# tszalay/poreseq

Measured on AMD Instinct MI355X. Metric: kb consensus refined/sec at 10x coverage, higher is better.
Workload: dtype f64; 1 GPU; poreseq consensus, 10 kb region, 10x synthetic coverage (BASELINE configs[1]), full Mutate.py schedule per region; a step is 280 independent regions per GPU = 14 lock-step batches; the batches of the timed steps run step by step (a step's batches all finish before the next step's start) through 14 batch slots (host threads) per GPU; marshalling + H2D of the events, host greedy steps and D2H inside; region_bases=10000, events=10, regions_per_gpu=280, batches_in_flight=14, step_barrier=True, parallelism=280 regions x 1 GPU(s), 14 host thread(s) per GPU, no data-path collective

## Files before the change

### poreseq_amd/csrc/ps_api.cpp

```cpp
#include <algorithm>
#include <cmath>
#include <cstring>
#include <memory>

#include "ps_host.h"
#include "ps_sw.h"

using namespace ps;

struct ps_align { Align a; };
struct ps_muts { std::vector<Mut> v; };
struct ps_seqs { std::vector<std::string> v; };
struct ps_rng { RandState* s = nullptr; ~ps_rng() { if (s) rand_state_free(s); } };

#define NEED_RT()            \
    Runtime* rt = nullptr;   \
    PS_TRY(runtime(&rt))

extern "C" {

const char* ps_last_error(void) { return last_error(); }
const char* ps_backend_name(void) { return "hip-gfx950"; }
int ps_info(char* out, int64_t cap) {
    if (!out || cap <= 0) return fail(PS_ERR_BAD_ARG, "ps_info");
// ... 458 lines not shown
    std::vector<std::unique_ptr<ps_seqs>> s(n);
    std::vector<VitReq> rq(n);
    for (int i = 0; i < n; i++) { s[i].reset(new ps_seqs()); rq[i].a = as[i]; rq[i].rng = (rng && rng[i]) ? rng[i]->s : nullptr; rq[i].out = &s[i]->v; }
    VitCall call;
    call.nkeep = nkeep; call.skip = skip; call.stay = stay; call.mmin = mmin; call.mmax = mmax;
    PS_TRY(viterbi_mutate(nullptr, call, rq.data(), rq.size()));
    for (int i = 0; i < n; i++) out[i] = s[i].release();
    return PS_OK;
}

int ps_swfull(const char* s1, int64_t n1, const char* s2, int64_t n2, int32_t* score, double* acc,
              int32_t* i1, int32_t* i2, int64_t cap, int64_t* np) {
    if (!s1 || !s2 || n1 < 0 || n2 < 0 || !np) return fail(PS_ERR_BAD_ARG, "ps_swfull");
    NEED_RT();
    int sc = 0; double ac = 0;
    std::vector<int> a, b;
    PS_TRY(sw_device(rt, std::string(s1, n1), std::string(s2, n2), &sc, &ac, &a, &b));
    if ((int64_t)a.size() > cap) return fail(PS_ERR_BAD_ARG, "ps_swfull: index capacity too small");
    if (score) *score = sc;
    if (acc) *acc = ac;
    for (size_t k = 0; k < a.size(); k++) { if (i1) i1[k] = a[k]; if (i2) i2[k] = b[k]; }
    *np = (int64_t)a.size();
    return PS_OK;
}
int ps_batch_sw_summary(int64_t n, const char* const* seq1, const int64_t* n1, const char* const* seq2, const int64_t* n2,
                        ps_sw_summary* out) {
    if (n < 0 || (n && (!seq1 || !n1 || !seq2 || !n2 || !out))) return fail(PS_ERR_BAD_ARG, "ps_batch_sw_summary");
    for (int64_t k = 0; k < n; k++)
        if (n1[k] < 0 || n2[k] < 0 || (n1[k] && !seq1[k]) || (n2[k] && !seq2[k])) return fail(PS_ERR_BAD_ARG, "ps_batch_sw_summary: bad pair");
    if (!n) return PS_OK;
    NEED_RT();
    std::vector<std::string> s(2 * (size_t)n);
    SwInput in;
    for (int64_t k = 0; k < n; k++) {
        if (n1[k]) s[2 * k].assign(seq1[k], (size_t)n1[k]);
        if (n2[k]) s[2 * k + 1].assign(seq2[k], (size_t)n2[k]);
    }
    for (int64_t k = 0; k < n; k++) in.push_back({&s[2 * k], &s[2 * k + 1]});
    std::vector<SwResult> res;
    PS_TRY(sw_summaries(rt, in, &res));
    for (int64_t k = 0; k < n; k++) {
        const SwResult& r = res[k];
        ps_sw_summary& o = out[k];
        o.score = r.score; o.n_pairs = r.n_pairs; o.n_match = r.n_match;
        o.first1 = r.first1; o.first2 = r.first2; o.last1 = r.last1; o.last2 = r.last2;
        o.gap1 = r.gap1; o.gap2 = r.gap2;
        o.accuracy = r.accuracy;
    }
    return PS_OK;
}
int ps_seq_to_states(const char* seq, int64_t n, int32_t* st, int64_t* ns) {
    if (!seq || n < 0 || !ns) return fail(PS_ERR_BAD_ARG, "ps_seq_to_states");
    std::vector<int> v = states_of(std::string(seq, n));
    if (st) std::copy(v.begin(), v.end(), st);
    *ns = (int64_t)v.size();
    return PS_OK;
}

int ps_debug_sw_band(int64_t* out) {
    if (!out) return fail(PS_ERR_BAD_ARG, "ps_debug_sw_band");
    sw_band_counters(out);
    return PS_OK;
}
int ps_debug_posterior(ps_align* a, int32_t e, double* main, double* stay) {
    if (!a || e < 0 || e >= a->a.E || !main) return fail(PS_ERR_BAD_ARG, "ps_debug_posterior");
    if (!a->a.nonfinite.empty()) return fail(PS_ERR_BAD_ARG, "ps_debug_posterior: " + a->a.nonfinite);
    NEED_RT();
    return debug_posterior(rt, &a->a, e, main, stay);
}
int ps_debug_fill(ps_align* a, int32_t e, int32_t dir, double* main, double* stay, uint8_t* sm, uint8_t* ss) {
    if (!a || e < 0 || e >= a->a.E || !main || dir < 0 || dir > 1) return fail(PS_ERR_BAD_ARG, "ps_debug_fill");
    NEED_RT();
    return debug_fill(rt, &a->a, e, dir, main, stay, sm, ss);
}
int ps_debug_poison(uint32_t index_word, uint64_t value_word, ps_poison_report* report, int32_t cap, int32_t* n_report) {
    if (cap < 0 || (cap && !report)) return fail(PS_ERR_BAD_ARG, "ps_debug_poison");
    NEED_RT();
    return debug_poison(rt, index_word, value_word, report, cap, n_report);
}
int ps_debug_viterbi(int32_t n, ps_align* const* a, int32_t build, int32_t nkeep, double skip, double stay, double mmin, double mmax,
                     int64_t cap_T, int32_t* T, double* obs, int16_t* bp, double* lik_final, double* fwd, int16_t* paths) {
    std::vector<Align*> as;
    PS_TRY(batch_handles(n, a, &as));
    if (nkeep < 0 || build < 0 || build > 3 || cap_T < 0 || (n && !T)) return fail(PS_ERR_BAD_ARG, "ps_debug_viterbi");
    return debug_viterbi(as, build, nkeep, skip, stay, mmin, mmax, cap_T, T, obs, bp, lik_final, fwd, paths);
}
int ps_debug_viterbi_steps(int32_t R, const int32_t* T, const double* obs, const double* rnd, int32_t nkeep, double skip, double stay,
                           double mmin, double mmax, int16_t* bp, double* lik_final, double* fwd, int16_t* paths) {
    if (R < 0 || nkeep < 0 || (R && !T)) return fail(PS_ERR_BAD_ARG, "ps_debug_viterbi_steps");
    int64_t ttot = 0;
    for (int r = 0; r < R; r++) { if (T[r] < 0) return fail(PS_ERR_BAD_ARG, "ps_debug_viterbi_steps: negative T"); ttot += T[r]; }
    if (ttot && (!obs || (nkeep && !rnd))) return fail(PS_ERR_BAD_ARG, "ps_debug_viterbi_steps: null rows or deviates");
    NEED_RT();
    return debug_viterbi_steps(rt, R, T, obs, rnd, nkeep, skip, stay, mmin, mmax, bp, lik_final, fwd, paths);
}

int ps_srand(uint32_t seed) { rand_seed(seed); return PS_OK; }
int ps_rand_draw(int64_t n, double* out) {
    if (n < 0 || (n && !out)) return fail(PS_ERR_BAD_ARG, "ps_rand_draw");
    for (int64_t k = 0; k < n; k++) out[k] = rand_next() / (double(RAND_MAX) + 1);
    return PS_OK;
}

int ps_set_sweep_min(int32_t n) { sweep_min_set(n); return PS_OK; }
int ps_set_sweep2_min(int32_t n) { sweep2_min_set(n); return PS_OK; }
int ps_set_sparse_min(int32_t n) { sparse_min_set(n); return PS_OK; }
int ps_set_device_fraction(double f) {
    if (f > 1.0) return fail(PS_ERR_BAD_ARG, "ps_set_device_fraction: a fraction in (0, 1]; <= 0 restores the default");
    device_fraction_set(f);
    return PS_OK;
}
int ps_set_sweep_form(int32_t K, int32_t NW) {
    if (K <= 0 && NW > 0 && NW != 1 && NW != 2 && NW != 4) return fail(PS_ERR_BAD_ARG, "ps_set_sweep_form: 1, 2 or 4 wavefronts per sweep");
    if (K > 0 && !sweep_form_exists(K, NW)) return fail(PS_ERR_BAD_ARG, "ps_set_sweep_form: no such form (rows per lane, wavefronts)");
    sweep_form_set(K, NW);
    return PS_OK;
}

int ps_prof_enable(int32_t on) {
    NEED_RT();
    prof_flush(rt);
    rt->prof_on = on != 0;
    rt->prof_defer = on == 2;
    return PS_OK;
}
int ps_prof_reset(void) {
    NEED_RT();
    prof_flush(rt);
    rt->prof.clear();
    return PS_OK;
}
int ps_prof_get(const char* name, double* ms, int64_t* n, double* bytes) {
    NEED_RT();
    prof_flush(rt);
    Prof p;
    if (name) { auto it = rt->prof.find(name); if (it != rt->prof.end()) p = it->second; }
    if (ms) *ms = p.ms;
    if (n) *n = p.launches;
    if (bytes) *bytes = p.bytes;
    return PS_OK;
}

int ps_prof_units(const char* name, double* units) {
    NEED_RT();
    prof_flush(rt);
    Prof p;
    if (name) { auto it = rt->prof.find(name); if (it != rt->prof.end()) p = it->second; }
    if (units) *units = p.units;
    return PS_OK;
}

}
```

### poreseq_amd/csrc/ps_internal.h

```cpp
#ifndef PS_INTERNAL_H_
#define PS_INTERNAL_H_

#include <hip/hip_runtime.h>
#include <stdint.h>

#include <map>
#include <string>
#include <type_traits>
#include <vector>

#include "../../include/poreseq_hip.h"
#include "ps_greedy.h"
#include "ps_editplan.h"
#include "ps_plan.h"

namespace ps {

constexpr double BIG = 1e300;

int fail(int code, const std::string& msg);
bool trace_on();
#define PS_HIP(expr)                                                                          \
    do {                                                                                      \
        hipError_t _e = (expr);                                                               \
// ... 201 lines not shown
struct GenoArgs {
    int nfrac;
    double f[GENO_MAX_FRAC], g[GENO_MAX_FRAC];
    double* score;
    double* lik;
    int* ncover;
};
constexpr int LINK_MAX_WINDOW = 8;
constexpr int PHASE_MAX_SETS = 8;
struct PhaseArgs {
    int W;
    int S;
    double min_link;
    double* score;
    ps_edit_link* link;
    ps_edit_phase* phase;
    ps_event_hap* hap;
    int* nsets;
};
enum class EditKind { List, Points, Support, Genotype, Phase };
struct ScoreLaunch {
    EditKind kind = EditKind::List;
    std::vector<ScoreArgs> sas; std::vector<PointArgs> pts; std::vector<SupportArgs> sps; std::vector<GenoArgs> gts; std::vector<PhaseArgs> phs;
    const ScoreArgs* d_sas = nullptr; const PointArgs* d_pts = nullptr; const SupportArgs* d_sps = nullptr; const GenoArgs* d_gts = nullptr;
    const PhaseArgs* d_phs = nullptr;
};
int launch_score(Runtime* rt, const BatchD& b, const ScoreLaunch& L);
int launch_begin(Runtime* rt, const BatchD& b);
int launch_gather_best(Runtime* rt, const BatchD& b, double* out);

struct StatJob {
    const double* ra;
    const double* mean;
    const double* model;
    const int* st;
    int n, S;
    const double* stdv;
    int grp, pad;
};
struct StatRegion { int job0, njobs, ngroups, tab0; };
int launch_align_stats(Runtime* rt, const StatJob* d_jobs, const StatRegion* d_regs, int nregs, int maxE, double alg_bytes, ps_event_stats* d_out);
constexpr int KMER_TILE = 512;
constexpr int KMER_BLOCKS = 4;
int launch_kmer_stats(Runtime* rt, const StatJob* d_jobs, const StatRegion* d_regs, int nregs, int maxG, double alg_bytes, ps_kmer_cell* d_out);
struct MoveJob {
    const long long* rec;
    const JobOut* out;
    uint8_t* step;
    int32_t* col;
    int n, pad;
};
struct MoveRun {
    const MoveJob* jobs = nullptr;
    const StatRegion* regs = nullptr;
    int nregs = 0, maxE = 0;
    ps_event_moves* out = nullptr;
    double alg_bytes = 0.0;
};
int launch_move_stats(Runtime* rt, const MoveRun& mv);

struct PostJob {
    double* emit;
    double* col;
    double* row;
};
constexpr int POST_MAX_SLOTS = 1024;
int launch_post(Runtime* rt, const BatchD& b, int P, const PostJob* d_jobs, ps_event_posterior* d_out, double cells);

int sw_device(Runtime* rt, const std::string& s1, const std::string& s2, int* score, double* accuracy,
              std::vector<int>* inds1, std::vector<int>* inds2);
void sw_band_counters(int64_t out[5]);

struct VitReg {
    const double* model;
    int E, T;
    int64_t in_off;
    int64_t t_off;
};
struct VitRegionH {
    int E = 0, T = 0;
    int index = -1;
    const double* obsin = nullptr;
    const double* d_model = nullptr;
    void* rng = nullptr;
    void (*draw)(void* rng, double* out , size_t n) = nullptr;
    std::vector<int16_t> paths;
};
struct VitTap {
    int obs_build = 0;
    const double* obs_rows = nullptr;
    std::vector<int> T;
    std::vector<double> obs;
    std::vector<short> bp;
    std::vector<double> lik_final;
    std::vector<double> fwd;
    std::vector<std::vector<int16_t>> paths;
};
bool vit_obs_lds_ok();
void launch_vit_obs(Runtime* rt, int build, const VitReg* d_regs, const int* d_posreg, const double* d_in, int64_t ttot, int maxE, double* d_obs, double* d_eobs);
int launch_vit_steps(Runtime* rt, const VitReg* d_regs, int R, const double* d_obs, const double* d_eobs, double skip, double stay, short* d_bp, double* d_fwd,
                     double* d_lik, bool keep_fwd);
int launch_vit_trace(Runtime* rt, const VitReg* d_regs, int R, int64_t ttot, int nkeep, double* d_fwd, const int* d_start, double skip, double stay,
                     const double* d_att, const double* d_rnd, short* d_path);

void prof_flush(Runtime* rt);
void prof_begin(Runtime* rt);
void prof_end(Runtime* rt, const char* name, double alg_bytes);

}

#endif
```

### poreseq_amd/csrc/ps_vit.cpp

```cpp
#include <algorithm>
#include <cmath>
#include <cstdlib>
#include <cstring>

#include "ps_host.h"
#include "ps_vitgather.h"
#include "ps_vitpath.h"

namespace ps {

inline int succ(int st, int k, int j) { return ((st << (2 * j)) & (NS - 1)) + k; }
inline char base_at(int st, int k) { return "ACGT"[3 & (st >> (2 * (4 - k)))]; }

static std::string path_to_bases(const int16_t* st, size_t len) {
    std::string s;
    int cur = st[0];
    s.push_back(base_at(cur, 0));
    for (size_t i = 1; i < len; i++) {
        if (cur == st[i]) continue;
        bool hit = false;
        for (int n = 1; n <= 4 && !hit; n++)
            for (int k = 0; k < (1 << (2 * n)); k++)
                if (succ(cur, k, n) == st[i]) {
                    for (int b = 1; b <= n; b++) s.push_back(base_at(cur, b));
// ... 28 lines not shown
void rand_state_free(RandState* r) { delete r; }
void rand_state_seed(RandState* r, unsigned seed) { rs_seed(r, seed); }
int rand_state_next(RandState* r) { return rs_next(r ? r : &t_rand); }

static void vit_draw(void* rng, double* rnd, size_t n) {
    RandState* r = (RandState*)rng;
    for (size_t k = 0; k < n; k++) rnd[k] = rand_state_next(r) / (double(RAND_MAX) + 1);
}

namespace {
struct Vit {
    Runtime* rt;
    const VitCall& call;
    VitReq* reqs;
    int R;
    Tick tk;
    std::vector<double*> h_ri;
    std::vector<JobOut*> info;
    std::vector<VitGather> gath;
    std::vector<VitRegionH> regs;
    Vit(Runtime* rt_, const VitCall& call_, VitReq* reqs_, size_t n) : rt(rt_), call(call_), reqs(reqs_), R((int)n), tk("viterbi_mutate") {}
    std::string named(int r) const { return std::string(call.who) + ": " + (call.lockstep ? "region " + std::to_string(r) + ": " : std::string()); }
};
}

static int check_call(const VitCall& c, const VitReq* reqs, size_t n) {
    const std::string who(c.who);
    if (c.nkeep < 0) return fail(PS_ERR_BAD_ARG, c.lockstep ? who + ": nkeep" : who);
    for (size_t k = 0; k < n; k++) if (reqs[k].a->E == 0) return fail(PS_ERR_BAD_ARG, c.lockstep ? who + ": no events" : who);
    for (size_t k = 0; k < n; k++) {
        const Align& a = *reqs[k].a;
        if (!a.nonfinite.empty())
            return fail(PS_ERR_BAD_ARG, who + ": " + a.nonfinite + " (ViterbiMutate needs finite levels with stdv > 0 and a model with positive deviations)");
    }
    return PS_OK;
}

static int refs_to_host(Vit& v) {
    v.h_ri.assign(v.R, nullptr);
    v.info.assign(v.R, nullptr);
    for (int r = 0; r < v.R; r++) {
        Align* a = v.reqs[r].a;
        PS_TRY(a->refs_to_host_async(v.rt));
        a->last_stream = (void*)v.rt->stream;
        PS_TRY(v.rt->down(&v.h_ri[r], a->d_ri, (size_t)a->ntot));
        PS_TRY(v.rt->down(&v.info[r], a->d_out, (size_t)a->E));
    }
    PS_HIP(hipStreamSynchronize(v.rt->stream));
    for (int r = 0; r < v.R; r++) v.reqs[r].a->refs_finish();
    v.tk.lap("refs D2H");
    return PS_OK;
}

static int check_refs(const Vit& v) {
    for (int r = 0; r < v.R; r++) {
        const Align& a = *v.reqs[r].a;
        for (int e = 0; e < a.E; e++) {
            const double* ra = a.h_ra.data() + a.off[e];
            for (int t = 0; t < a.n[e]; t++)
                if (ra[t] >= 2147483648.0) {
                    char val[64];
                    snprintf(val, sizeof(val), "%g", ra[t]);
                    return fail(PS_ERR_BAD_ARG, v.named(r) + "event " + std::to_string(e) + ", level " + std::to_string(t) + ": ref_align = " + val +
                                                    " is not below 2^31 (ViterbiMutate walks the positions from (int)ref_align)");
                }
        }
    }
    return PS_OK;
}

static void gather(Vit& v) {
    v.gath.resize(v.R);
    par_for(v.R, [&](int r) {
        const Align* a = v.reqs[r].a;
        std::vector<VitGatherEvent> ev(a->E);
        for (int e = 0; e < a->E; e++) ev[e] = {a->n[e], a->off[e], v.info[r][e].has_index != 0, v.info[r][e].refstart, v.info[r][e].refend};
        vit_gather({a->E, ev.data(), a->h_ra.data(), v.h_ri[r], a->h_mean.data(), a->h_stdv.data()}, &v.gath[r]);
    });
    v.tk.lap("gather levels");
    v.regs.resize(v.R);
    for (int r = 0; r < v.R; r++) {
        VitRegionH& g = v.regs[r];
        g.E = v.reqs[r].a->E; g.T = v.gath[r].T; g.obsin = v.gath[r].obsin.data(); g.d_model = v.reqs[r].a->d_model;
        g.rng = v.reqs[r].rng; g.draw = vit_draw;
        g.index = v.call.lockstep ? r : -1;
    }
}

static int in_sub_batches(Vit& v) {
    auto need = [&](size_t k) { return 26.0 * 1024.0 * (double)v.regs[k].T + 32.0 * (double)v.regs[k].T * v.regs[k].E; };
    double cap = std::max(PLAN_VITERBI_FLOOR, PLAN_VITERBI_FRAC * device_share_bytes());
    for (size_t k0 = 0; k0 < v.regs.size();) {
        const size_t k1 = greedy_cut(k0, v.regs.size(), cap, (size_t)-1, need);
        const int rc = viterbi_batch(v.rt, v.call, v.regs.data() + k0, k1 - k0);
        if (rc == PS_ERR_NOMEM && k1 - k0 > 1) { cap *= 0.5; continue; }
        PS_TRY(rc);
        k0 = k1;
    }
    v.tk.lap("device");
    return PS_OK;
}

static void to_bases(Vit& v) {
    par_for(v.R, [&](int r) {
        const VitRegionH& g = v.regs[r];
        for (size_t at = 0; at < g.paths.size(); at += (size_t)g.T) v.reqs[r].out->push_back(path_to_bases(g.paths.data() + at, (size_t)g.T));
    });
    v.tk.lap("paths to bases");
}

int viterbi_mutate(Runtime* rt, const VitCall& call, VitReq* reqs, size_t n) {
    PS_TRY(check_call(call, reqs, n));
    if (!rt) PS_TRY(runtime(&rt));
    Vit v(rt, call, reqs, n);
    for (int r = 0; r < v.R; r++) reqs[r].out->clear();
    PS_TRY(refs_to_host(v));
    PS_TRY(check_refs(v));
    gather(v);
    PS_TRY(in_sub_batches(v));
    to_bases(v);
    return PS_OK;
}

namespace {
struct VitBatch {
    Runtime* rt;
    const VitCall& call;
    VitRegionH* regions;
    int R;
    VitTap* tap;
    std::vector<VitReg> regs;
    std::vector<int> pos_reg;
    int64_t ttot = 0, intot = 0;
    int maxE = 0;
    size_t b_obs = 0, b_fwd = 0, b_bp = 0;
    VitReg* d_regs = nullptr;
    int* d_posreg = nullptr;
    double *d_in = nullptr, *d_obs = nullptr, *d_eobs = nullptr, *d_fwd = nullptr, *d_lik = nullptr;
    short* d_bp = nullptr;
    double *lik = nullptr, *tap_obs = nullptr, *tap_fwd = nullptr, *h_rand = nullptr;
    short* tap_bp = nullptr;
    std::vector<int> starts;
    VitBatch(Runtime* rt_, const VitCall& call_, VitRegionH* regions_, size_t n) : rt(rt_), call(call_), regions(regions_), R((int)n), tap(call_.tap) {}
    size_t cells() const { return (size_t)ttot * NS; }
};
}

static void plan(VitBatch& b) {
    b.regs.resize(b.R);
    for (int r = 0; r < b.R; r++) {
        const VitRegionH& g = b.regions[r];
        b.regions[r].paths.clear();
        b.regs[r].model = g.d_model; b.regs[r].E = g.E; b.regs[r].T = g.T;
        b.regs[r].in_off = b.intot; b.regs[r].t_off = b.ttot;
        b.intot += (int64_t)g.T * g.E * 4; b.ttot += g.T;
        b.maxE = std::max(b.maxE, g.E);
    }
    if (b.tap)
        for (int r = 0; r < b.R; r++) { b.tap->T.push_back(b.regions[r].T); b.tap->paths.emplace_back(); b.tap->lik_final.insert(b.tap->lik_final.end(), NS, 0.0); }
    if (b.ttot <= 0) return;
    b.pos_reg.resize((size_t)b.ttot);
    for (int r = 0; r < b.R; r++) std::fill(b.pos_reg.begin() + b.regs[r].t_off, b.pos_reg.begin() + b.regs[r].t_off + b.regs[r].T, r);
    auto al = [](size_t x) { return (x + 255) & ~(size_t)255; };
    b.b_obs = al(b.cells() * sizeof(double));
    b.b_fwd = al((size_t)(b.call.nkeep ? b.ttot : 1) * NS * sizeof(double));
    b.b_bp = al(b.cells() * sizeof(short));
}

static int place(VitBatch& b) {
    Runtime* rt = b.rt;
    const int nkeep = b.call.nkeep;
    PS_TRY(rt->buf("vit_regs").ensure(b.R * sizeof(VitReg)));
    PS_TRY(rt->buf("vit_posreg").ensure((size_t)b.ttot * sizeof(int)));
    PS_TRY(rt->buf("vit_in").ensure((size_t)std::max<int64_t>(b.intot, 1) * sizeof(double)));
    DBuf& arena = rt->buf("rec");
    PS_TRY(arena.ensure(2 * b.b_obs + b.b_fwd + b.b_bp));
    PS_TRY(rt->buf("vit_lik").ensure((size_t)b.R * NS * sizeof(double)));
    if (nkeep > 0) {
        PS_TRY(rt->buf("vit_att").ensure(nkeep * sizeof(double)));
        PS_TRY(rt->buf("vit_start").ensure(b.R * sizeof(int)));
        PS_TRY(rt->buf("vit_rnd").ensure((size_t)nkeep * b.ttot * sizeof(double)));
        PS_TRY(rt->buf("vit_path").ensure((size_t)nkeep * b.ttot * sizeof(short)));
    }
    b.d_regs = rt->buf("vit_regs").as<VitReg>();
    b.d_posreg = rt->buf("vit_posreg").as<int>();
    b.d_in = rt->buf("vit_in").as<double>();
    char* abase = (char*)arena.p;
    b.d_obs = (double*)abase;
    b.d_eobs = (double*)(abase + b.b_obs);
    b.d_fwd = (double*)(abase + 2 * b.b_obs);
    b.d_bp = (short*)(abase + 2 * b.b_obs + b.b_fwd);
    b.d_lik = rt->buf("vit_lik").as<double>();
    return PS_OK;
}

static int upload(VitBatch& b) {
    PS_TRY(b.rt->up(b.d_regs, b.regs.data(), b.R * sizeof(VitReg)));
    PS_TRY(b.rt->up(b.d_posreg, b.pos_reg.data(), (size_t)b.ttot * sizeof(int)));
    for (int r = 0; r < b.R; r++) {
        const VitRegionH& g = b.regions[r];
        if (g.T && g.E) PS_TRY(b.rt->up(b.d_in + b.regs[r].in_off, g.obsin, (size_t)g.T * g.E * 4 * sizeof(double)));
    }
    return PS_OK;
}

static int emissions(VitBatch& b) {
    const bool lds_ok = b.maxE <= 72 && vit_obs_lds_ok();
    int build = lds_ok ? 1 : b.maxE <= 64 ? 2 : 3;
    if (b.tap && b.tap->obs_build) {
        build = b.tap->obs_build;
        if (build < 1 || build > 3 || (build == 1 && !lds_ok) || (build == 2 && b.maxE > 64))
            return fail(PS_ERR_BAD_ARG, "ViterbiMutate: the emission build asked for does not take this many events");
    }
    prof_begin(b.rt);
    if (b.tap && b.tap->obs_rows) {
        std::vector<double> eo(b.cells());
        for (size_t k = 0; k < eo.size(); k++) eo[k] = std::exp(b.tap->obs_rows[k]);
        PS_TRY(b.rt->up(b.d_obs, b.tap->obs_rows, eo.size() * sizeof(double)));
        PS_TRY(b.rt->up(b.d_eobs, eo.data(), eo.size() * sizeof(double)));
    } else {
        launch_vit_obs(b.rt, build, b.d_regs, b.d_posreg, b.d_in, b.ttot, b.maxE, b.d_obs, b.d_eobs);
    }
    return PS_OK;
}

static int steps(VitBatch& b) {
    PS_TRY(launch_vit_steps(b.rt, b.d_regs, b.R, b.d_obs, b.d_eobs, b.call.skip, b.call.stay, b.d_bp, b.d_fwd, b.d_lik, b.call.nkeep != 0));
    return b.rt->down(&b.lik, b.d_lik, (size_t)b.R * NS);
}

static int tap_tables(VitBatch& b) {
    if (!b.tap) return PS_OK;
    PS_TRY(b.rt->down(&b.tap_obs, b.d_obs, b.cells()));
    PS_TRY(b.rt->down(&b.tap_bp, b.d_bp, b.cells()));
    if (b.call.nkeep > 0) PS_TRY(b.rt->down(&b.tap_fwd, b.d_fwd, b.cells()));
    return PS_OK;
}
static void tap_append(VitBatch& b) {
    VitTap* tap = b.tap;
    if (!tap) return;
    tap->obs.insert(tap->obs.end(), b.tap_obs, b.tap_obs + b.cells());
    tap->bp.insert(tap->bp.end(), b.tap_bp, b.tap_bp + b.cells());
    if (b.tap_fwd) tap->fwd.insert(tap->fwd.end(), b.tap_fwd, b.tap_fwd + b.cells());
    for (int r = 0; r < b.R; r++)
        if (b.regions[r].T) std::copy(b.lik + (size_t)r * NS, b.lik + (size_t)(r + 1) * NS, tap->lik_final.end() - (size_t)(b.R - r) * NS);
}
static void tap_paths(VitBatch& b) {
    if (b.tap) for (int r = 0; r < b.R; r++) *(b.tap->paths.end() - b.R + r) = b.regions[r].paths;
}

static int draw(VitBatch& b) {
    const int nkeep = b.call.nkeep;
    if (nkeep > 0) {
        b.h_rand = (double*)b.rt->stage.alloc((size_t)nkeep * b.ttot * sizeof(double));
        if (!b.h_rand) return fail(PS_ERR_NOMEM, "hipHostMalloc (staging arena)");
        for (int r = 0; r < b.R; r++) b.regions[r].draw(b.regions[r].rng, b.h_rand + (size_t)nkeep * b.regs[r].t_off, (size_t)nkeep * b.regions[r].T);
    }
    PS_HIP(hipStreamSynchronize(b.rt->stream));
    tap_append(b);
    b.starts.assign(b.R, 0);
    for (int r = 0; r < b.R; r++) b.starts[r] = (int)(std::max_element(b.lik + (size_t)r * NS, b.lik + (size_t)(r + 1) * NS) - (b.lik + (size_t)r * NS));
    return PS_OK;
}

static int follow_tail(VitBatch& b) {
    short* bp = nullptr;
    PS_TRY(b.rt->down(&bp, b.d_bp, b.cells()));
    PS_HIP(hipStreamSynchronize(b.rt->stream));
    prof_end(b.rt, "viterbi", (double)b.ttot * NS * (8.0 * b.maxE + 8 + 2));
    for (int r = 0; r < b.R; r++) {
        VitRegionH& g = b.regions[r];
        if (!g.T) continue;
        std::vector<int> p(g.T);
        const int64_t dead = vit_follow_bp(bp, b.regs[r].t_off, g.T, NS, b.starts[r], p.data());
        if (dead >= 0) {
            for (int q = 0; q < b.R; q++) b.regions[q].paths.clear();
            return fail(PS_ERR_BAD_ARG, std::string(b.call.who) + ": " + (g.index >= 0 ? "region " + std::to_string(g.index) + ": " : std::string()) +
                                            "no state is reachable at kept position " + std::to_string(dead) +
                                            " (every emission there is -inf or below -1e300, or the running scores have passed -1e300)");
        }
        g.paths.assign(p.begin(), p.end());
    }
    tap_paths(b);
    return PS_OK;
}

static int trace_tail(VitBatch& b) {
    Runtime* rt = b.rt;
    const int nkeep = b.call.nkeep;
    std::vector<double> att(nkeep);
    for (int k = 0; k < nkeep; k++) att[k] = b.call.mmin + (b.call.mmax - b.call.mmin) * k / (double)nkeep;
    PS_TRY(rt->up(rt->buf("vit_att").p, att.data(), nkeep * sizeof(double)));
    PS_TRY(rt->up(rt->buf("vit_start").p, b.starts.data(), b.R * sizeof(int)));
    PS_HIP(hipMemcpyAsync(rt->buf("vit_rnd").p, b.h_rand, (size_t)nkeep * b.ttot * sizeof(double), hipMemcpyHostToDevice, rt->stream));
    PS_TRY(launch_vit_trace(rt, b.d_regs, b.R, b.ttot, nkeep, b.d_fwd, rt->buf("vit_start").as<int>(), b.call.skip, b.call.stay, rt->buf("vit_att").as<double>(),
// ... 29 lines not shown
```

### poreseq_amd/csrc/ps_viterbi.hip

```cpp
#include <atomic>

#include "ps_internal.h"

namespace ps {

struct ModelRowV { double mu, sg, lsg, sm, lam, llam; };
__device__ __forceinline__ double emission_v(const ModelRowV& m, double x, double sd, double lsd, double log2pi) {
    double d = (x - m.mu) / m.sg;
    double l = -0.5 * (d * d + log2pi) - m.lsg;
    double e = (sd - m.sm) / m.sm;
    l += 0.5 * (m.llam - 3 * lsd - log2pi - e * e * m.lam / sd);
    return l;
}

template <int VMAXE>
__global__ __launch_bounds__(256) void k_vit_obs(const VitReg* __restrict__ regs, const int* __restrict__ pos_reg, const double* __restrict__ obsin,
                                                 double log2pi, double* __restrict__ obs, double* __restrict__ eobs) {
    const int t = blockIdx.x;
    const VitReg R = regs[pos_reg[t]];
    const int E = R.E;
    const double* in = obsin + R.in_off + (size_t)(t - R.t_off) * E * 4;
    for (int st = threadIdx.x; st < NS; st += 256) {
        double v[VMAXE];
        int nl = 0;
        for (int e = 0; e < E; e++) {
            if (in[e * 4 + 3] == 0.0) continue;
            const double* gm = R.model + (size_t)e * 6 * NS;
            ModelRowV m = {gm[st], gm[NS + st], gm[2 * NS + st], gm[3 * NS + st], gm[4 * NS + st], gm[5 * NS + st]};
            const double l = emission_v(m, in[e * 4 + 0], in[e * 4 + 1], in[e * 4 + 2], log2pi);
            int k = nl++;
            while (k > 0 && v[k - 1] > l) { v[k] = v[k - 1]; k--; }
            v[k] = l;
        }
        double r;
        if (nl > 1) {
            int drop = (int)floor(nl * 0.25);
            if (drop > nl - 2) drop = 0;
            double s = 0.0;
            for (int k = drop; k < nl; k++) s += v[k];
            r = s / (double)(nl - drop);
        } else {
            r = nl == 1 ? v[0] : 0.0;
        }
        obs[(size_t)t * NS + st] = r;
        eobs[(size_t)t * NS + st] = exp(r);
    }
}

__global__ __launch_bounds__(256) void k_vit_obs_lds(const VitReg* __restrict__ regs, const int* __restrict__ pos_reg, const double* __restrict__ obsin,
                                                     double log2pi, double* __restrict__ obs, double* __restrict__ eobs) {
    extern __shared__ double vit_v[];
    const int t = blockIdx.x;
    const VitReg R = regs[pos_reg[t]];
    const int E = R.E;
    const double* in = obsin + R.in_off + (size_t)(t - R.t_off) * E * 4;
    double* v = vit_v + threadIdx.x;
    for (int st = threadIdx.x; st < NS; st += 256) {
        int nl = 0;
        for (int e = 0; e < E; e++) {
            if (in[e * 4 + 3] == 0.0) continue;
            const double* gm = R.model + (size_t)e * 6 * NS;
            ModelRowV m = {gm[st], gm[NS + st], gm[2 * NS + st], gm[3 * NS + st], gm[4 * NS + st], gm[5 * NS + st]};
            const double l = emission_v(m, in[e * 4 + 0], in[e * 4 + 1], in[e * 4 + 2], log2pi);
            int k = nl++;
            while (k > 0) {
                const double w = v[(k - 1) * 256];
                if (!(w > l)) break;
                v[k * 256] = w;
                k--;
            }
            v[k * 256] = l;
        }
        double r;
        if (nl > 1) {
            int drop = (int)floor(nl * 0.25);
            if (drop > nl - 2) drop = 0;
            double s = 0.0;
            for (int k = drop; k < nl; k++) s += v[k * 256];
            r = s / (double)(nl - drop);
        } else {
            r = nl == 1 ? v[0] : 0.0;
        }
        obs[(size_t)t * NS + st] = r;
        eobs[(size_t)t * NS + st] = exp(r);
    }
}

#define PS_LDS_BARRIER() asm volatile("s_waitcnt lgkmcnt(0)\n\ts_barrier" ::: "memory")

struct Fam { double mx, second, psum; int idx; int pad; };

__device__ __forceinline__ Fam fam_join(const Fam& A, const Fam& B) {
    Fam r;
    r.mx = fmax(A.mx, B.mx);
    const int ia = A.mx == r.mx ? A.idx : 0x7fffffff, ib = B.mx == r.mx ? B.idx : 0x7fffffff;
    r.idx = min(ia, ib);
    const double lower = A.mx == B.mx ? -BIG * 10 : fmin(A.mx, B.mx);
    r.second = fmax(fmax(A.second, B.second), lower);
    r.psum = A.psum + B.psum;
    r.pad = 0;
    return r;
}

template <int N>
__device__ __forceinline__ double row_shl(double v) {
    int lo = __double2loint(v), hi = __double2hiint(v);
    lo = __builtin_amdgcn_update_dpp(0, lo, 0x100 + N, 0xf, 0xf, true);
    hi = __builtin_amdgcn_update_dpp(0, hi, 0x100 + N, 0xf, 0xf, true);
    return __hiloint2double(hi, lo);
}
template <int N>
__device__ __forceinline__ Fam fam_shl(const Fam& f) {
    Fam o;
    o.mx = row_shl<N>(f.mx); o.second = row_shl<N>(f.second); o.psum = row_shl<N>(f.psum);
    o.idx = __builtin_amdgcn_update_dpp(0, f.idx, 0x100 + N, 0xf, 0xf, true); o.pad = 0;
    return o;
}
__device__ __forceinline__ double wave_sum(double v) {
    v += row_shl<1>(v); v += row_shl<2>(v); v += row_shl<4>(v); v += row_shl<8>(v);
    auto lane_d = [&](int l) {
        const int lo = __builtin_amdgcn_readlane(__double2loint(v), l), hi = __builtin_amdgcn_readlane(__double2hiint(v), l);
        return __hiloint2double(hi, lo);
    };
    return (lane_d(0) + lane_d(16)) + (lane_d(32) + lane_d(48));
}

__device__ __forceinline__ double below(double x) {
    long long b = __double_as_longlong(x);
    b += x < 0.0 ? 1 : -1;
    return __longlong_as_double(b);
}

#define VPAD(q) ((q) + ((q) >> 5))

__global__ __launch_bounds__(1024) void k_vit_steps(const VitReg* __restrict__ regs, const double* __restrict__ obs_all, const double* __restrict__ eobs_all,
                                                    double skip, double stay, double lskip, double lstay, double l25,
                                                    short* __restrict__ bp_all, double* __restrict__ lfwd_all,
                                                    double* __restrict__ lik_final_all, int keep_fwd) {
    const int T = regs[blockIdx.x].T;
    const size_t roff = (size_t)regs[blockIdx.x].t_off * NS;
    const double* __restrict__ obs = obs_all + roff;
    const double* __restrict__ eobs = eobs_all + roff;
    short* __restrict__ bp = bp_all + roff;
    double* __restrict__ lfwd_out = lfwd_all + (keep_fwd ? roff : 0);
    double* __restrict__ lik_final = lik_final_all + (size_t)blockIdx.x * NS;
    if (T <= 0) return;
    __shared__ double s_lik[2][NS + NS / 32], s_fwd[2][NS + NS / 32];
    __shared__ Fam s_fam[336];
    __shared__ double s_red[16];
    __shared__ double s_scale;
    const int c = threadIdx.x, lane = c & 63, wave = c >> 6;
    s_lik[0][VPAD(c)] = 0.0;
    s_fwd[0][VPAD(c)] = 1.0 / NS;
    if (c == 0) s_scale = 1.0;
    if (c < 16) s_red[c] = 1.0 / 16;
    __syncthreads();
    const double sp1 = 0.25, sp2 = sp1 * 0.25 * skip, sp3 = sp2 * 0.25 * skip;
    const double lsp1 = l25, lsp2 = lsp1 + l25 + lskip, lsp3 = lsp2 + l25 + lskip;
    int fj = 0, fg = 0, fq0 = 0, fqs = 0;
    if (c < 256) { fj = 1; fg = c; fq0 = c; fqs = 256; }
    else if (c < 512) { const int u = c - 256; fj = 2; fg = u >> 2; fq0 = fg + 256 * (u & 3); fqs = 64; }
    else if (c < 768) { const int u = c - 512; fj = 3; fg = u >> 4; fq0 = fg + 64 * (u & 15); fqs = 16; }
    int cur = 0;
    constexpr int VPF = 4;
    double oA[VPF], eA[VPF], oB[VPF], eB[VPF];
    const int TL = T - 1;
#define VIT_LOAD(O, E, t0)                                             \
// ... 17 lines not shown
            }
            Fam f = fam_join(fam_join(m[0], m[1]), fam_join(m[2], m[3]));
            if (fj >= 2) { f = fam_join(f, fam_shl<1>(f)); f = fam_join(f, fam_shl<2>(f)); }
            if (fj == 3) { f = fam_join(f, fam_shl<4>(f)); f = fam_join(f, fam_shl<8>(f)); }
            const bool writer = fj == 1 || (fj == 2 && (c & 3) == 0) || (fj == 3 && (c & 15) == 0);
            if (writer) s_fam[(fj == 1 ? 0 : fj == 2 ? 256 : 320) + fg] = f;
        } else if (c == 1023) {
            double ptot = 0.0;
            for (int w = 0; w < 16; w++) ptot += s_red[w];
            int ex;
            frexp(ptot, &ex);
            s_scale = ldexp(1.0, min(-ex, 1000));
        }
        PS_LDS_BARRIER();
        double best = -BIG; int bq = -1; double fsum = 0.0;
#pragma unroll
        for (int j = 1; j <= 3; j++) {
            const int g = j == 1 ? (c >> 2) : j == 2 ? (c >> 4) : (c >> 6);
            const Fam f = s_fam[(j == 1 ? 0 : j == 2 ? 256 : 320) + g];
            const double a = o + (j == 1 ? lsp1 : j == 2 ? lsp2 : lsp3);
            const double m = a + f.mx;
            fsum += (j == 1 ? sp1 : j == 2 ? sp2 : sp3) * f.psum;
            if (f.second > -BIG * 5 && a + f.second == m) {
                const int cnt = 1 << (2 * j), sh = 10 - 2 * j;
                for (int k = 0; k < cnt; k++) {
                    const int q = g + (k << sh);
                    const double l = a + pl[VPAD(q)];
                    if (l > best) { best = l; bq = q; }
                }
            } else if (m > best) { best = m; bq = f.idx; }
        }
        {
            const double l = o + lstay + pl[VPAD(c)];
            if (l > best) { best = l; bq = c; }
            fsum += stay * pf[VPAD(c)];
        }
        const double nf = (fsum * s_scale) * eo;
        {
            const double wsum = wave_sum(nf);
            if (lane == 0) s_red[wave] = wsum;
        }
        s_lik[cur ^ 1][VPAD(c)] = best;
        s_fwd[cur ^ 1][VPAD(c)] = nf;
        bp[(size_t)t * NS + c] = (short)bq;
        if (keep_fwd) lfwd_out[(size_t)t * NS + c] = nf;
        PS_LDS_BARRIER();
        cur ^= 1;
    };
    VIT_LOAD(oA, eA, 0)
    for (int t0 = 0; t0 < T; t0 += 2 * VPF) {
        VIT_LOAD(oB, eB, t0 + VPF)
        VIT_RUN(oA, eA, t0)
        VIT_LOAD(oA, eA, t0 + 2 * VPF)
        VIT_RUN(oB, eB, t0 + VPF)
    }
#undef VIT_LOAD
#undef VIT_RUN
    lik_final[c] = s_lik[cur][VPAD(c)];
}

__device__ __forceinline__ double trans_weight(int cur, int p, double skip, double stay) {
    double t = 0.0, sp = 0.25;
#pragma unroll
    for (int j = 1; j <= 4; j++) {
        if ((p & ((1 << (10 - 2 * j)) - 1)) == (cur >> (2 * j))) t += sp;
        sp = sp * 0.25 * skip;
    }
    if (p == cur) t = stay;
    return t;
}

__global__ void k_vit_log(double* __restrict__ v, size_t n) {
    const size_t i = (size_t)blockIdx.x * blockDim.x + threadIdx.x;
    if (i < n) v[i] = log(v[i]);
}

template <int N>
__device__ __forceinline__ double row_shr(double v) {
    int lo = __double2loint(v), hi = __double2hiint(v);
    lo = __builtin_amdgcn_update_dpp(0, lo, 0x110 + N, 0xf, 0xf, true);
    hi = __builtin_amdgcn_update_dpp(0, hi, 0x110 + N, 0xf, 0xf, true);
    return __hiloint2double(hi, lo);
}
__device__ __forceinline__ double lane_get(double v, int l) {
    return __hiloint2double(__builtin_amdgcn_readlane(__double2hiint(v), l), __builtin_amdgcn_readlane(__double2loint(v), l));
}
__device__ __forceinline__ double wave_scan(double v, int lane) {
    v += row_shr<1>(v); v += row_shr<2>(v); v += row_shr<4>(v); v += row_shr<8>(v);
    const double t0 = lane_get(v, 15), t1 = lane_get(v, 31), t2 = lane_get(v, 47);
    const int row = lane >> 4;
    const double add = row == 0 ? 0.0 : row == 1 ? t0 : row == 2 ? t0 + t1 : (t0 + t1) + t2;
    return v + add;
}

constexpr int VT_THREADS = 512;
constexpr int VT_SPT = NS / VT_THREADS;
constexpr int VT_WAVES = VT_THREADS / 64;
__global__ __launch_bounds__(VT_THREADS) void k_vit_trace(const VitReg* __restrict__ regs, const double* __restrict__ lfwd_all, const int* __restrict__ starts,
                                                         double skip, double stay, const double* __restrict__ atten,
                                                         const double* __restrict__ rnd_all, short* __restrict__ path_all) {
    const int T = regs[blockIdx.y].T;
    if (T <= 0) return;
    const int start = starts[blockIdx.y];
    const double* __restrict__ lfwd = lfwd_all + (size_t)regs[blockIdx.y].t_off * NS;
    const double* __restrict__ rnd = rnd_all + (size_t)gridDim.x * regs[blockIdx.y].t_off;
    short* __restrict__ path = path_all + (size_t)gridDim.x * regs[blockIdx.y].t_off;
    __shared__ double s_wtot[2][VT_WAVES];
    __shared__ int s_pick[2][VT_WAVES];
    const int k = blockIdx.x, t = threadIdx.x, l = t & 63, w = t >> 6;
    const double at = atten[k];
    int cur = start;
    double2 lf = *(const double2*)(lfwd + (size_t)(T - 1) * NS + VT_SPT * t);
    double ex0 = exp(at * lf.x), ex1 = exp(at * lf.y);
    double rcur = rnd[(size_t)k * T];
    for (int i = T - 1; i >= 0; i--) {
        const int par = i & 1;
        if (t == 0) path[(size_t)k * T + i] = (short)cur;
        double2 nx = lf;
        double rnx = rcur;
        if (i > 0) { nx = *(const double2*)(lfwd + (size_t)(i - 1) * NS + VT_SPT * t); rnx = rnd[(size_t)k * T + (T - i)]; }
        const double tv0 = trans_weight(cur, VT_SPT * t, skip, stay), tv1 = trans_weight(cur, VT_SPT * t + 1, skip, stay);
        const double c0 = tv0 == 0.0 ? 0.0 : tv0 * ex0;
        const double c1 = c0 + (tv1 == 0.0 ? 0.0 : tv1 * ex1);
        const double nex0 = exp(at * nx.x), nex1 = exp(at * nx.y);
        const double incl = wave_scan(c1, l);
        if (l == 63) s_wtot[par][w] = incl;
        PS_LDS_BARRIER();
        double before = 0.0, total = 0.0;
#pragma unroll
        for (int q = 0; q < VT_WAVES; q++) {
            const double wq = s_wtot[par][q];
            if (q == w) before = total;
            total = q ? total + wq : wq;
        }
        const double base = before + (incl - c1);
        const double thr = rcur * total;
        int pick = 0x7fffffff;
        if (thr < base + c1) pick = thr < base + c0 ? VT_SPT * t : VT_SPT * t + 1;
        const unsigned long long hit = __builtin_amdgcn_ballot_w64(pick != 0x7fffffff);
        int wpick = 0x7fffffff;
        if (hit) wpick = __builtin_amdgcn_readlane(pick, __builtin_ctzll(hit));
        if (l == 0) s_pick[par][w] = wpick;
        PS_LDS_BARRIER();
        int pk = 0x7fffffff;
#pragma unroll
        for (int q = VT_WAVES - 1; q >= 0; q--) { const int pq = s_pick[par][q]; pk = pq != 0x7fffffff ? pq : pk; }
        cur = pk == 0x7fffffff ? NS - 1 : pk;
        lf = nx; rcur = rnx; ex0 = nex0; ex1 = nex1;
    }
}


bool vit_obs_lds_ok() {
    static std::atomic<int> attr(0);
    if (attr.load(std::memory_order_acquire) == 0) {
        const hipError_t e = hipFuncSetAttribute((const void*)k_vit_obs_lds, hipFuncAttributeMaxDynamicSharedMemorySize, 160 * 1024);
        if (e != hipSuccess) (void)hipGetLastError();
        attr.store(e == hipSuccess ? 1 : -1, std::memory_order_release);
    }
    return attr.load(std::memory_order_acquire) == 1;
}

void launch_vit_obs(Runtime* rt, int build, const VitReg* d_regs, const int* d_posreg, const double* d_in, int64_t ttot, int maxE, double* d_obs, double* d_eobs) {
    if (rt->prof_on) rt->prof[build == 1 ? "vit_obs_lds" : (build == 2 ? "vit_obs_64" : "vit_obs_256")].launches++;
    if (build == 1)
        hipLaunchKernelGGL(k_vit_obs_lds, dim3((unsigned)ttot), dim3(256), (size_t)256 * std::max(maxE, 1) * sizeof(double), rt->stream, d_regs, d_posreg, d_in,
                           std::log(2 * M_PI), d_obs, d_eobs);
    else if (build == 2) hipLaunchKernelGGL(k_vit_obs<64>, dim3((unsigned)ttot), dim3(256), 0, rt->stream, d_regs, d_posreg, d_in, std::log(2 * M_PI), d_obs, d_eobs);
    else hipLaunchKernelGGL(k_vit_obs<256>, dim3((unsigned)ttot), dim3(256), 0, rt->stream, d_regs, d_posreg, d_in, std::log(2 * M_PI), d_obs, d_eobs);
}

int launch_vit_steps(Runtime* rt, const VitReg* d_regs, int R, const double* d_obs, const double* d_eobs, double skip, double stay, short* d_bp, double* d_fwd,
                     double* d_lik, bool keep_fwd) {
    hipLaunchKernelGGL(k_vit_steps, dim3(R), dim3(1024), 0, rt->stream, d_regs, d_obs, d_eobs, skip, stay, std::log(skip), std::log(stay),
                       std::log(0.25), d_bp, d_fwd, d_lik, keep_fwd ? 1 : 0);
    PS_LAUNCH_CHECK();
    return PS_OK;
}

int launch_vit_trace(Runtime* rt, const VitReg* d_regs, int R, int64_t ttot, int nkeep, double* d_fwd, const int* d_start, double skip, double stay,
                     const double* d_att, const double* d_rnd, short* d_path) {
    hipLaunchKernelGGL(k_vit_log, dim3((unsigned)(((size_t)ttot * NS + 255) / 256)), dim3(256), 0, rt->stream, d_fwd, (size_t)ttot * NS);
    hipLaunchKernelGGL(k_vit_trace, dim3(nkeep, R), dim3(VT_THREADS), 0, rt->stream, d_regs, d_fwd, d_start, skip, stay, d_att, d_rnd, d_path);
    PS_LAUNCH_CHECK();
    return PS_OK;
}

}
```

Before: 252.9 kb/s.

## Add chunked Viterbi emission kernel reusing model rows across timesteps

Adds a new emission kernel in which each block handles several consecutive timesteps (P) of a region. Each model row is loaded once per event and reused across those timesteps, and each lane keeps a register sorting network for the trimmed mean. Per-event 1/sd values are computed once per chunk and broadcast with readlane, and divisions become reciprocal multiplies when the alignment's fastdiv flag allows it. The new path is chosen by default when every region admits fastdiv and there are at most 12 events. The cost is higher register pressure and template instantiations, plus slightly different rounding from the reciprocal divides.

```diff
diff --git a/poreseq_amd/csrc/ps_api.cpp b/poreseq_amd/csrc/ps_api.cpp
--- a/poreseq_amd/csrc/ps_api.cpp
+++ b/poreseq_amd/csrc/ps_api.cpp
@@ -564,7 +564,7 @@
                      int64_t cap_T, int32_t* T, double* obs, int16_t* bp, double* lik_final, double* fwd, int16_t* paths) {
     std::vector<Align*> as;
     PS_TRY(batch_handles(n, a, &as));
-    if (nkeep < 0 || build < 0 || build > 3 || cap_T < 0 || (n && !T)) return fail(PS_ERR_BAD_ARG, "ps_debug_viterbi");
+    if (nkeep < 0 || build < 0 || build > 4 || cap_T < 0 || (n && !T)) return fail(PS_ERR_BAD_ARG, "ps_debug_viterbi");
     return debug_viterbi(as, build, nkeep, skip, stay, mmin, mmax, cap_T, T, obs, bp, lik_final, fwd, paths);
 }
 int ps_debug_viterbi_steps(int32_t R, const int32_t* T, const double* obs, const double* rnd, int32_t nkeep, double skip, double stay,
diff --git a/poreseq_amd/csrc/ps_internal.h b/poreseq_amd/csrc/ps_internal.h
--- a/poreseq_amd/csrc/ps_internal.h
+++ b/poreseq_amd/csrc/ps_internal.h
@@ -307,6 +307,7 @@
     int index = -1;
     const double* obsin = nullptr;
     const double* d_model = nullptr;
+    bool fastdiv = false;
     void* rng = nullptr;
     void (*draw)(void* rng, double* out , size_t n) = nullptr;
     std::vector<int16_t> paths;
@@ -322,6 +323,7 @@
     std::vector<std::vector<int16_t>> paths;
 };
 bool vit_obs_lds_ok();
+int vit_obs_chunk_len(int maxE);
 void launch_vit_obs(Runtime* rt, int build, const VitReg* d_regs, const int* d_posreg, const double* d_in, int64_t ttot, int maxE, double* d_obs, double* d_eobs);
 int launch_vit_steps(Runtime* rt, const VitReg* d_regs, int R, const double* d_obs, const double* d_eobs, double skip, double stay, short* d_bp, double* d_fwd,
                      double* d_lik, bool keep_fwd);
diff --git a/poreseq_amd/csrc/ps_vit.cpp b/poreseq_amd/csrc/ps_vit.cpp
--- a/poreseq_amd/csrc/ps_vit.cpp
+++ b/poreseq_amd/csrc/ps_vit.cpp
@@ -134,6 +134,7 @@
     for (int r = 0; r < v.R; r++) {
         VitRegionH& g = v.regs[r];
         g.E = v.reqs[r].a->E; g.T = v.gath[r].T; g.obsin = v.gath[r].obsin.data(); g.d_model = v.reqs[r].a->d_model;
+        g.fastdiv = v.reqs[r].a->fastdiv;
         g.rng = v.reqs[r].rng; g.draw = vit_draw;
         g.index = v.call.lockstep ? r : -1;
     }
@@ -258,11 +259,17 @@
 
 static int emissions(VitBatch& b) {
     const bool lds_ok = b.maxE <= 72 && vit_obs_lds_ok();
-    int build = lds_ok ? 1 : b.maxE <= 64 ? 2 : 3;
+    bool fastdiv = true;
+    for (int r = 0; r < b.R; r++) fastdiv = fastdiv && b.regions[r].fastdiv;
+    const bool chunk_ok = fastdiv && vit_obs_chunk_len(b.maxE) > 0;
+    int build = chunk_ok ? 4 : lds_ok ? 1 : b.maxE <= 64 ? 2 : 3;
     if (b.tap && b.tap->obs_build) {
         build = b.tap->obs_build;
-        if (build < 1 || build > 3 || (build == 1 && !lds_ok) || (build == 2 && b.maxE > 64))
+        if (build < 1 || build > 4 || (build == 1 && !lds_ok) || (build == 2 && b.maxE > 64))
             return fail(PS_ERR_BAD_ARG, "ViterbiMutate: the emission build asked for does not take this many events");
+        if (build == 4 && !chunk_ok)
+            return fail(PS_ERR_BAD_ARG, fastdiv ? "ViterbiMutate: the emission build asked for does not take this many events"
+                                                : "ViterbiMutate: the emission build asked for divides by reciprocal, which these tables do not admit");
     }
     prof_begin(b.rt);
     if (b.tap && b.tap->obs_rows) {
diff --git a/poreseq_amd/csrc/ps_viterbi.hip b/poreseq_amd/csrc/ps_viterbi.hip
--- a/poreseq_amd/csrc/ps_viterbi.hip
+++ b/poreseq_amd/csrc/ps_viterbi.hip
@@ -1,6 +1,6 @@
 #include <atomic>
 
-#include "ps_internal.h"
+#include "ps_dev.h"
 
 namespace ps {
 
@@ -83,6 +83,93 @@
         }
         obs[(size_t)t * NS + st] = r;
         eobs[(size_t)t * NS + st] = exp(r);
+    }
+}
+
+__device__ __forceinline__ double lane_get(double v, int l) {
+    return __hiloint2double(__builtin_amdgcn_readlane(__double2hiint(v), l), __builtin_amdgcn_readlane(__double2loint(v), l));
+}
+
+__device__ __forceinline__ double emission_r(const ModelRowV& m, double rsg, double rsm, double x, double sd, double lsd, double rsd, double log2pi) {
+    double d = mdiv(x - m.mu, m.sg, rsg);
+    double l = -0.5 * (d * d + log2pi) - m.lsg;
+    double e = mdiv(sd - m.sm, m.sm, rsm);
+    l += 0.5 * (m.llam - 3 * lsd - log2pi - mdiv(e * e * m.lam, sd, rsd));
+    return l;
+}
+
+__device__ __forceinline__ ModelRowV model_row(const double* model, int e, int st) {
+    const double* gm = model + (size_t)e * 6 * NS;
+    return {gm[st], gm[NS + st], gm[2 * NS + st], gm[3 * NS + st], gm[4 * NS + st], gm[5 * NS + st]};
+}
+template <int P, int ME>
+__global__ __launch_bounds__(256) void k_vit_obs_chunk(const VitReg* __restrict__ regs, const int* __restrict__ pos_reg, const double* __restrict__ obsin,
+                                                       int64_t ttot, double log2pi, double* __restrict__ obs, double* __restrict__ eobs) {
+    static_assert(P * ME <= 128, "1 / sd of a chunk in two registers per lane");
+    const int lane = threadIdx.x & 63;
+    int64_t t = (int64_t)blockIdx.x * P;
+    const int64_t tend = t + P < ttot ? t + P : ttot;
+    while (t < tend) {
+        const VitReg R = regs[pos_reg[t]];
+        const int E = R.E < ME ? R.E : ME;
+        const int64_t rend = R.t_off + R.T;
+        const int n = (int)((tend < rend ? tend : rend) - t);
+        const double* in = obsin + R.in_off + (size_t)(t - R.t_off) * R.E * 4;
+        const int ne = n * E;
+        const double rs0 = lane < ne ? 1.0 / in[lane * 4 + 1] : 0.0;
+        const double rs1 = lane + 64 < ne ? 1.0 / in[(lane + 64) * 4 + 1] : 0.0;
+        for (int st = threadIdx.x; st < NS; st += 256) {
+            double v[P][ME];
+            int nl[P];
+#pragma unroll
+            for (int p = 0; p < P; p++) {
+                nl[p] = 0;
+#pragma unroll
+                for (int k = 0; k < ME; k++) v[p][k] = HUGE_VAL;
+            }
+            ModelRowV nx = model_row(R.model, 0, st);
+#pragma unroll
+            for (int e = 0; e < ME; e++) {
+                if (e >= E) continue;
+                const ModelRowV m = nx;
+                if (e + 1 < E) nx = model_row(R.model, e + 1, st);
+                const double rsg = 1.0 / m.sg, rsm = 1.0 / m.sm;
+#pragma unroll
+                for (int p = 0; p < P; p++) {
+                    const int i = p * E + e;
+                    if (p >= n || in[i * 4 + 3] == 0.0) continue;
+                    const double rsd = i < 64 ? lane_get(rs0, i) : lane_get(rs1, i - 64);
+                    double l = emission_r(m, rsg, rsm, in[i * 4 + 0], in[i * 4 + 1], in[i * 4 + 2], rsd, log2pi);
+#pragma unroll
+                    for (int k = 0; k < ME; k++) {
+                        if (k > e) continue;
+                        const double lo = fmin(v[p][k], l);
+                        l = fmax(v[p][k], l);
+                        v[p][k] = lo;
+                    }
+                    nl[p]++;
+                }
+            }
+#pragma unroll
+            for (int p = 0; p < P; p++) {
+                if (p >= n) continue;
+                const int c = nl[p];
+                double r;
+                if (c > 1) {
+                    int drop = (int)floor(c * 0.25);
+                    if (drop > c - 2) drop = 0;
+                    double s = 0.0;
+#pragma unroll
+                    for (int k = 0; k < ME; k++) if (k >= drop && k < c) s += v[p][k];
+                    r = s / (double)(c - drop);
+                } else {
+                    r = c == 1 ? v[p][0] : 0.0;
+                }
+                obs[(size_t)(t + p) * NS + st] = r;
+                eobs[(size_t)(t + p) * NS + st] = exp(r);
+            }
+        }
+        t += n;
     }
 }
 
@@ -266,9 +353,6 @@
     hi = __builtin_amdgcn_update_dpp(0, hi, 0x110 + N, 0xf, 0xf, true);
     return __hiloint2double(hi, lo);
 }
-__device__ __forceinline__ double lane_get(double v, int l) {
-    return __hiloint2double(__builtin_amdgcn_readlane(__double2hiint(v), l), __builtin_amdgcn_readlane(__double2loint(v), l));
-}
 __device__ __forceinline__ double wave_scan(double v, int lane) {
     v += row_shr<1>(v); v += row_shr<2>(v); v += row_shr<4>(v); v += row_shr<8>(v);
     const double t0 = lane_get(v, 15), t1 = lane_get(v, 31), t2 = lane_get(v, 47);
@@ -345,9 +429,24 @@
     return attr.load(std::memory_order_acquire) == 1;
 }
 
+int vit_obs_chunk_len(int maxE) { return maxE < 1 ? 0 : maxE <= 4 ? 8 : maxE <= 8 ? 4 : maxE <= 12 ? 2 : 0; }
+
+template <int P, int ME>
+static void launch_vit_obs_chunk(Runtime* rt, const VitReg* d_regs, const int* d_posreg, const double* d_in, int64_t ttot, double* d_obs, double* d_eobs) {
+    hipLaunchKernelGGL((k_vit_obs_chunk<P, ME>), dim3((unsigned)((ttot + P - 1) / P)), dim3(256), 0, rt->stream, d_regs, d_posreg, d_in, ttot, std::log(2 * M_PI),
+                       d_obs, d_eobs);
+}
+
 void launch_vit_obs(Runtime* rt, int build, const VitReg* d_regs, const int* d_posreg, const double* d_in, int64_t ttot, int maxE, double* d_obs, double* d_eobs) {
-    if (rt->prof_on) rt->prof[build == 1 ? "vit_obs_lds" : (build == 2 ? "vit_obs_64" : "vit_obs_256")].launches++;
-    if (build == 1)
+    if (rt->prof_on) {
+        rt->prof[build == 1 || build == 4 ? "vit_obs_lds" : (build == 2 ? "vit_obs_64" : "vit_obs_256")].launches++;
+        if (build == 4) rt->prof["vit_obs_chunk"].launches++;
+    }
+    if (build == 4) {
+        if (maxE <= 4) launch_vit_obs_chunk<8, 4>(rt, d_regs, d_posreg, d_in, ttot, d_obs, d_eobs);
+        else if (maxE <= 8) launch_vit_obs_chunk<4, 8>(rt, d_regs, d_posreg, d_in, ttot, d_obs, d_eobs);
+        else launch_vit_obs_chunk<2, 12>(rt, d_regs, d_posreg, d_in, ttot, d_obs, d_eobs);
+    } else if (build == 1)
         hipLaunchKernelGGL(k_vit_obs_lds, dim3((unsigned)ttot), dim3(256), (size_t)256 * std::max(maxE, 1) * sizeof(double), rt->stream, d_regs, d_posreg, d_in,
                            std::log(2 * M_PI), d_obs, d_eobs);
     else if (build == 2) hipLaunchKernelGGL(k_vit_obs<64>, dim3((unsigned)ttot), dim3(256), 0, rt->stream, d_regs, d_posreg, d_in, std::log(2 * M_PI), d_obs, d_eobs);
```

After: 256.7 kb/s (median of 6 runs). +1.5%, better.
